# YujiaoShi/HighlyAccurate

Measured on AMD Instinct MI355X. Metric: image-pairs/sec through N-iter LM pose loop, KITTI shapes, higher is better.
Workload: dtype bf16; 1 GPU; BASELINE configs[1]: LM_S2GP.forward(mode='test'), sat 512x512, grd 256x1024, VGG-16 two-branch, level 3, 5 LM iters x 3 levels, 3-DoF, random-init weights; pairs_per_gpu=32, global_batch=32, parallelism=batch-sharded x1, no collective

## Files before the change

### highlyaccurate_amd/csrc/common.h

```cpp
#pragma once
#include <hip/hip_runtime.h>
#include <atomic>
#include <stdarg.h>
#include <stdio.h>
#include "../../include/hla.h"

void hla_set_error(const char* fmt, ...);

enum { K_PACK = 0, K_CONV02, K_CONV_NT2, K_CONV_NT2_POOL, K_CONV_NT1, K_CONV_NT1_POOL, K_CONF, K_L2NORM,
       K_LM256, K_LM128, K_LM64, K_LM16, K_LMSOLVE, K_GRIDSAMPLE, K_LMBWD, K_WGRAD, K_ELEMWISE };
void hla_prof_begin(int id, double flops, double bytes, hipStream_t st);
void hla_prof_begin_dyn(int id, double flops, double bytes, hipStream_t st, const int* dev_live, int denom);
void hla_prof_end(hipStream_t st);
bool hla_prof_on();

#ifndef HLA_CONV_STAMPS
#define HLA_CONV_STAMPS 0
#endif
#if HLA_CONV_STAMPS
constexpr int HLA_STAMP_N = 8;
struct HlaStampCfg { unsigned long long* buf; int want; int counter; unsigned grid_x, grid_y; };
extern HlaStampCfg g_hla_stamp;
#endif

#define HLA_CHECK_HIP(expr)                                                              \
  do {                                                                                   \
    hipError_t _e = (expr);                                                              \
    if (_e != hipSuccess) {                                                              \
      hla_set_error("%s failed: %s (%s:%d)", #expr, hipGetErrorString(_e), __FILE__, __LINE__); \
      return HLA_ERR_HIP;                                                                \
    }                                                                                    \
  } while (0)

static inline bool hla_dtype_ok(int dtype) { return dtype == HLA_F32 || dtype == HLA_BF16 || dtype == HLA_F16 || dtype == HLA_F16X3; }

#define HLA_REQUIRE(cond, ...)      \
  do {                              \
    if (!(cond)) {                  \
      hla_set_error(__VA_ARGS__);   \
      return HLA_ERR_ARG;           \
    }                               \
  } while (0)

struct HlaPerDeviceOnce {
  std::atomic<unsigned long long> mask{0};
  template <typename F> hipError_t run(F&& f) {
    int d = 0;
    (void)hipGetDevice(&d);
    const unsigned long long bit = (d >= 0 && d < 64) ? 1ull << d : 0ull;
    if (mask.load(std::memory_order_acquire) & bit) return hipSuccess;
    const hipError_t e = f();
    if (e == hipSuccess) mask.fetch_or(bit, std::memory_order_release);
    return e;
  }
};

static inline size_t hla_align_up(size_t x, size_t a) { return (x + a - 1) / a * a; }

__device__ __forceinline__ float wave_sum_f32(float v) {
#pragma unroll
  for (int o = 32; o > 0; o >>= 1) v += __shfl_xor(v, o, 64);
  return v;
}
__device__ __forceinline__ double wave_sum_f64(double v) {
#pragma unroll
  for (int o = 32; o > 0; o >>= 1) v += __shfl_xor(v, o, 64);
  return v;
}
```

### highlyaccurate_amd/csrc/lm_solve.hip

```cpp
#include "lm_common.h"
#include <cstring>
#include <mutex>

struct SolveArgs {
  const double* part;
  const double* sat_inv;
  const double* grd_inv;
  int nt, part_ld;
  float* pose;
  float* trace_out;
  int trace_stride;
  const float* rand_uv;
  double* normal_eq;
  double* coef;
  const float* R_FL;
  const float* T_FL;
  int B, reinit;
  int optimizer, t;
  double beta1, beta2;
  double* adam;
  const int* in_view;
  LmSolveCfg cfg;
  LmGeom next;
  unsigned* zero_ticket;
  int zero_steps, zero_pose;
  int* reach_clear;
  const int* gate;
};

template <bool COHERENT>
__device__ __forceinline__ void lm_solve_body(const SolveArgs& a, int b, int lane) {
  float su = a.pose[b * 3 + 0], sv = a.pose[b * 3 + 1], th = a.pose[b * 3 + 2];
  if (!a.part) {
    if (a.reach_clear && lane == 0) a.reach_clear[b] = 0;
    if (a.zero_ticket)
      for (int k = lane; k < a.zero_steps; k += 64) a.zero_ticket[(size_t)k * a.B + b] = 0u;
    if (a.zero_pose) {
      su = sv = th = 0.f;
      if (lane < 3) a.pose[b * 3 + lane] = 0.f;
    }
  }

  if (a.part) {
    double s[14];
#pragma unroll
    for (int k = 0; k < 14; ++k) s[k] = 0.0;
    for (int i = lane; i < a.nt; i += 64) {
      const double* p = a.part + ((size_t)b * a.part_ld + i) * PART_N;
#pragma unroll
      for (int k = 0; k < 14; ++k)
        s[k] += COHERENT ? __hip_atomic_load(p + k, __ATOMIC_RELAXED, __HIP_MEMORY_SCOPE_AGENT) : p[k];
    }
#pragma unroll
    for (int k = 0; k < 14; ++k) s[k] = wave_sum_f64(s[k]);

    if (lane == 0) {
      const double as = a.sat_inv ? a.sat_inv[b] : 1.0, ag = a.grd_inv ? a.grd_inv[b] : 1.0;
      s[0] *= as * as; s[1] *= ag * ag;
      for (int k = 2; k < 11; ++k) s[k] *= as * as;
      for (int k = 11; k < 14; ++k) s[k] *= as * ag;
      if (a.normal_eq) {
        for (int k = 0; k < 14; ++k) a.normal_eq[(size_t)b * 16 + k] = s[k];
        a.normal_eq[(size_t)b * 16 + 14] = a.in_view ? (double)a.in_view[b] : 0.0;
        a.normal_eq[(size_t)b * 16 + 15] = 0.0;
      }
      double H[3][3], g[3], Mi[3][3], d[3], ns, ng;
      if (a.optimizer == 0 || a.optimizer == 3) {
        lm_solve_step(a.cfg, s, H, g, Mi, d, ns, ng);
      } else {
        for (int p = 0; p < 3; ++p) d[p] = 2.0 * (s[8 + p] - s[11 + p]);
        if (a.optimizer == 2) {
          double* mv = a.adam + (size_t)b * 6;
          for (int p = 0; p < 3; ++p) {
            const double m = a.beta1 * mv[p] + (1.0 - a.beta1) * d[p];
            const double v = a.beta2 * mv[3 + p] + (1.0 - a.beta2) * d[p] * d[p];
            mv[p] = m; mv[3 + p] = v;
            d[p] = (m / (1.0 - pow(a.beta1, a.t + 1))) / (sqrt(v / (1.0 - pow(a.beta2, a.t + 1))) + 1e-8);
          }
        }
        for (int p = 0; p < 3; ++p) d[p] *= 0.01;
      }
      su = (float)((double)su - d[0]);
      sv = (float)((double)sv - d[1]);
      th = (float)((double)th - d[2]);
      if (a.reinit) {
        const float ru = a.rand_uv[b], rv = a.rand_uv[a.B + b];
        su = (su > -2.5f && su < 2.5f) ? su : ru;
        sv = (sv > -2.5f && sv < 2.5f) ? sv : rv;
      }
      a.pose[b * 3 + 0] = su; a.pose[b * 3 + 1] = sv; a.pose[b * 3 + 2] = th;
      float* tr = a.trace_out + (size_t)b * a.trace_stride;
      tr[0] = su; tr[1] = sv; tr[2] = th;
    }
  }
  if (a.coef && lane == 0)
    lm_coefficients(a.next, su, sv, th, a.R_FL ? a.R_FL + (size_t)b * 9 : nullptr, a.T_FL ? a.T_FL + (size_t)b * 3 : nullptr,
                    a.coef + (size_t)b * COEF_N);
}

__global__ __launch_bounds__(64) void lm_solve(SolveArgs a) {
  if (a.gate && a.gate[blockIdx.x] == 0) return;
  lm_solve_body<false>(a, blockIdx.x, threadIdx.x);
}

struct AccumArgs {
  const void* sat;
  const void* grd;
  const float* conf;
  LmPoints pts;
  const double* coef;
  double* part;
  int A, h, w, row0, npix, TP, nt, part_ld, xcd_affine;
  int b0, nb;
  int hs, rskip;
  const unsigned char* keep;
  unsigned* ticket;
  int col0;
  int* reach_flag;
  const int* gate;
};

typedef float lm_f2 __attribute__((ext_vector_type(2)));
template <typename F> __device__ __forceinline__ lm_f2 lm_pair(const uint4& v, int ep);
template <> __device__ __forceinline__ lm_f2 lm_pair<float>(const uint4& v, int ep) {
  lm_f2 r;
  r.x = __uint_as_float(ep == 0 ? v.x : v.z);
  r.y = __uint_as_float(ep == 0 ? v.y : v.w);
  return r;
}
template <> __device__ __forceinline__ lm_f2 lm_pair<__bf16>(const uint4& v, int ep) {
  const unsigned w = ep == 0 ? v.x : ep == 1 ? v.y : ep == 2 ? v.z : v.w;
  lm_f2 r;
  r.x = __uint_as_float(w << 16);
  r.y = __uint_as_float(w & 0xffff0000u);
  return r;
}
template <> __device__ __forceinline__ lm_f2 lm_pair<_Float16>(const uint4& v, int ep) {
  typedef _Float16 h2 __attribute__((ext_vector_type(2)));
  const unsigned w = ep == 0 ? v.x : ep == 1 ? v.y : ep == 2 ? v.z : v.w;
  const h2 h = __builtin_bit_cast(h2, w);
  lm_f2 r;
  r.x = (float)h[0];
  r.y = (float)h[1];
  return r;
}

#define LM_OCC 6
#define LM_UNROLL(F) (sizeof(F) == 4 ? 2 : 1)
#define FWD_MAX_TP 512
static inline int lm_pick_tile_fwd(int npix) { return npix >= 16384 ? 512 : (npix >= 4096 ? 256 : 128); }
template <int C, bool USE_W, typename F>
__global__ __launch_bounds__(256, LM_OCC) void lm_accum(AccumArgs a, SolveArgs sa) {
  __shared__ PixParam pp[FWD_MAX_TP];
  __shared__ float red[4][14];
  __shared__ double redd[14];
  int b, tile;
  if (!lm_block_map(a.xcd_affine, a.nt, a.nb, b, tile, a.b0)) return;
  if (a.gate && a.gate[b] == 0) return;
  const int t = threadIdx.x;
  const int p0 = tile * a.TP;
  const int np = min(a.TP, a.npix - p0);
  const double* cf = a.coef + (size_t)b * COEF_N;

  for (int tt = t; tt < np; tt += 256) {
    const int p = p0 + tt;
    const int r = a.row0 + p / a.w, c = p % a.w;
    const float cw = USE_W ? a.conf[((size_t)b * a.hs + (r - a.rskip)) * a.w + c] : 1.f;
    float q[3];
    const bool gm = lm_point(a.pts, b, r, c, a.w, q);
    const bool kept = !a.keep || a.keep[p];
    PixParam P = lm_pixel<C>(cf, q, gm, a.A, cw, a.col0, (a.reach_flag && kept) ? a.reach_flag + b : nullptr);
    if (!kept) {
      P.wx0 = P.wx1 = P.wy0 = P.wy1 = 0.f; P.off = a.col0 * C; P.dxo = P.dyo = 0; P.j2u = P.j2v = 0.f; P.gm = P.wt = P.m = 0.f;
    }
    pp[tt] = P;
  }
  __syncthreads();

  const float j0u = (float)cf[8], j0v = (float)cf[9], j1u = (float)cf[10], j1v = (float)cf[11];
  constexpr int EPL = 16 / (int)sizeof(F);
  constexpr int LPP = C / EPL;
  constexpr int PPW = 64 / LPP;
  const int lane = t & 63, wave = t >> 6;
  const int sub = lane / LPP, cl = (lane % LPP) * EPL;
  const F* satb = (const F*)a.sat + (size_t)b * a.A * a.A * C + cl;
  const F* grdb = (const F*)a.grd + ((size_t)b * a.hs * a.w + (size_t)(a.row0 - a.rskip) * a.w + p0) * C + cl;

  float aS = 0, aG = 0, T1 = 0, T2 = 0, T3 = 0, B1 = 0, B2 = 0, Q = 0, U1 = 0, U2 = 0, U3 = 0, V1 = 0, V2 = 0, V3 = 0;

  constexpr int UNR = LM_UNROLL(F);
#pragma unroll UNR
  for (int i = wave * PPW + sub; i < np; i += 4 * PPW) {
    const PixParam P = pp[i];
    const uint4 t00 = *(const uint4*)(satb + P.off);
    const uint4 t01 = *(const uint4*)(satb + P.off + P.dxo);
    const uint4 t10 = *(const uint4*)(satb + P.off + P.dyo);
    const uint4 t11 = *(const uint4*)(satb + P.off + P.dyo + P.dxo);
    const uint4 gg = *(const uint4*)(grdb + (size_t)i * C);
    lm_f2 xx = {0.f, 0.f}, xy = xx, yy = xx, xs = xx, ys = xx, xg = xx, yg = xx, ss2 = xx, gg2 = xx;
#pragma unroll
    for (int ep = 0; ep < EPL / 2; ++ep) {
      const lm_f2 c00 = lm_pair<F>(t00, ep), c01 = lm_pair<F>(t01, ep), c10 = lm_pair<F>(t10, ep), c11 = lm_pair<F>(t11, ep);
      const lm_f2 top = P.wx0 * c00 + P.wx1 * c01;
      const lm_f2 bot = P.wx0 * c10 + P.wx1 * c11;
      const lm_f2 s = P.wy0 * top + P.wy1 * bot;
      const lm_f2 dsy = bot - top;
      const lm_f2 dsx = P.wy0 * (c01 - c00) + P.wy1 * (c11 - c10);
      const lm_f2 g = lm_pair<F>(gg, ep) * P.gm;
      xx += dsx * dsx; xy += dsx * dsy; yy += dsy * dsy;
      xs += dsx * s; ys += dsy * s; xg += dsx * g; yg += dsy * g;
      ss2 += s * s; gg2 += g * g;
    }
    float Sxx = xx.x + xx.y, Sxy = xy.x + xy.y, Syy = yy.x + yy.y, Sxs = xs.x + xs.y, Sys = ys.x + ys.y;
    float Sxg = xg.x + xg.y, Syg = yg.x + yg.y;
    const float Sss = ss2.x + ss2.y, Sgg = gg2.x + gg2.y;
    aS += Sss; aG += Sgg;
    if (USE_W) { Sxx *= P.wt; Sxy *= P.wt; Syy *= P.wt; Sxs *= P.wt; Sys *= P.wt; Sxg *= P.wt; Syg *= P.wt; }
    T1 += Sxx; T2 += Sxy; T3 += Syy;
    const float b1 = P.j2u * Sxx + P.j2v * Sxy, b2 = P.j2u * Sxy + P.j2v * Syy;
    B1 += b1; B2 += b2;
    Q += P.j2u * b1 + P.j2v * b2;
    U1 += Sxs; U2 += Sys; U3 += P.j2u * Sxs + P.j2v * Sys;
    V1 += Sxg; V2 += Syg; V3 += P.j2u * Sxg + P.j2v * Syg;
  }

  float acc[14] = {aS, aG, T1, T2, T3, B1, B2, Q, U1, U2, U3, V1, V2, V3};
#pragma unroll
  for (int k = 0; k < 14; ++k) acc[k] = wave_sum_f32(acc[k]);
  if (lane == 0) {
#pragma unroll
    for (int k = 0; k < 14; ++k) red[wave][k] = acc[k];
  }
  __syncthreads();
  if (t < 14) redd[t] = ((double)red[0][t] + (double)red[1][t]) + ((double)red[2][t] + (double)red[3][t]);
  __syncthreads();
  if (wave != 0) return;
  if (t < PART_N) {
    const double au = (double)j0u, av = (double)j0v, bu = (double)j1u, bv = (double)j1v;
    const double t1 = redd[2], t2 = redd[3], t3 = redd[4], b1 = redd[5], b2 = redd[6];
    double v = 0.0;
    switch (t) {
      case 0: v = redd[0]; break;
      case 1: v = redd[1]; break;
      case 2: v = au * au * t1 + 2.0 * au * av * t2 + av * av * t3; break;
      case 3: v = au * bu * t1 + (au * bv + av * bu) * t2 + av * bv * t3; break;
      case 4: v = au * b1 + av * b2; break;
      case 5: v = bu * bu * t1 + 2.0 * bu * bv * t2 + bv * bv * t3; break;
      case 6: v = bu * b1 + bv * b2; break;
      case 7: v = redd[7]; break;
      case 8: v = au * redd[8] + av * redd[9]; break;
      case 9: v = bu * redd[8] + bv * redd[9]; break;
      case 10: v = redd[10]; break;
      case 11: v = au * redd[11] + av * redd[12]; break;
      case 12: v = bu * redd[11] + bv * redd[12]; break;
      case 13: v = redd[13]; break;
      default: break;
    }
    __hip_atomic_store(a.part + ((size_t)b * a.part_ld + tile) * PART_N + t, v, __ATOMIC_RELAXED, __HIP_MEMORY_SCOPE_AGENT);
  }
  const unsigned old = lm_draw_ticket(a.ticket + b, lane);
  if (old + 1 != (unsigned)a.nt) return;
  lm_solve_body<true>(sa, b, lane);
}

__global__ __launch_bounds__(256) void lm_inview_kernel(const double* __restrict__ coef, LmPoints pts, int w, int A,
                                                        int npix, int* __restrict__ count, int b0) {
  const int b = b0 + blockIdx.y, p = blockIdx.x * 256 + threadIdx.x;
  const double* cf = coef + (size_t)b * COEF_N;
  int in = 0;
  if (p < npix) {
    float q[3];
    (void)lm_point(pts, b, p / w, p % w, w, q);
    const double X = q[0], Y = q[1], Z = q[2];
    const double u = cf[0] * X + cf[1] * Y + cf[2] * Z + cf[3];
    const double v = cf[4] * X + cf[5] * Y + cf[6] * Z + cf[7];
    const double lim = (double)(A - 1);
    in = ((u >= 0.0) && (u <= lim) && (v >= 0.0) && (v <= lim)) ? 1 : 0;
  }
  const unsigned long long m = __ballot(in);
  if ((threadIdx.x & 63) == 0 && m) atomicAdd(count + b, __popcll(m));
}

static size_t ws_layout(const hla_s2g_config* cfg, const hla_s2g_level* lv, int B, size_t* off_coef, size_t* off_pose,
                        size_t* off_part, int* part_ld) {
  int max_nt = 1;
  for (int l = 0; l < cfg->n_levels; ++l) {
    const int npix = (lv[l].h - lv[l].row0) * lv[l].w;
    const int tp = lm_pick_tile_fwd(npix);
    max_nt = max(max_nt, (npix + tp - 1) / tp);
  }
  *part_ld = max_nt;
  size_t o = 0;
  *off_coef = o; o += hla_align_up((size_t)B * COEF_N * sizeof(double), 256);
  *off_pose = o; o += hla_align_up((size_t)B * 3 * sizeof(float), 256);
  *off_part = o; o += hla_align_up((size_t)B * max_nt * PART_N * sizeof(double), 256);
  o += hla_align_up((size_t)B * cfg->n_levels * cfg->n_iters * sizeof(unsigned), 256);
  o += hla_align_up((size_t)B * cfg->n_levels * cfg->n_iters * sizeof(int), 256);
  o += hla_align_up((size_t)B * 6 * sizeof(double), 256);
  return o;
}

extern "C" size_t hla_s2g_workspace_bytes(const hla_s2g_config* cfg, const hla_s2g_level* levels, int B) {
  size_t a, b, c;
  int ld;
  return ws_layout(cfg, levels, B, &a, &b, &c, &ld);
}

template <bool W, typename F>
static void launch_accum_f(int C, dim3 grid, hipStream_t st, const AccumArgs& a, const SolveArgs& sa) {
  switch (C) {
    case 256: hipLaunchKernelGGL((lm_accum<256, W, F>), grid, dim3(256), 0, st, a, sa); break;
    case 128: hipLaunchKernelGGL((lm_accum<128, W, F>), grid, dim3(256), 0, st, a, sa); break;
    case 64: hipLaunchKernelGGL((lm_accum<64, W, F>), grid, dim3(256), 0, st, a, sa); break;
    case 16: hipLaunchKernelGGL((lm_accum<16, W, F>), grid, dim3(256), 0, st, a, sa); break;
  }
}
template <bool W>
static void launch_accum(int C, int feat_dtype, dim3 grid, hipStream_t st, const AccumArgs& a, const SolveArgs& sa) {
  if (feat_dtype == HLA_BF16) launch_accum_f<W, __bf16>(C, grid, st, a, sa);
  else if (feat_dtype == HLA_F16) launch_accum_f<W, _Float16>(C, grid, st, a, sa);
  else launch_accum_f<W, float>(C, grid, st, a, sa);
}

int hla_s2g_validate(const char* who, const hla_s2g_config* cfg, const hla_s2g_level* lv, const float* R_FL,
                     const float* T_FL, int B) {
  HLA_REQUIRE(cfg && lv, "%s: null argument", who);
  HLA_REQUIRE(B > 0 && cfg->n_levels >= 1 && cfg->n_levels <= 4 && cfg->n_iters >= 1, "%s: bad sizes", who);
  HLA_REQUIRE(cfg->dof >= 1 && cfg->dof <= 3, "%s: dof must be 1..3", who);
  HLA_REQUIRE(cfg->proj == 0, "%s: cfg->proj selects the projection of hla_g2s_* only (must be 0 here)", who);
  HLA_REQUIRE(!cfg->ford || (R_FL && T_FL), "%s: Ford mode needs R_FL and T_FL", who);
  HLA_REQUIRE(cfg->reach_mode == 0 || (!strcmp(who, "hla_s2g_lm_solve") && cfg->reach_mode >= 1 && cfg->reach_mode <= 2 && cfg->reach_flag),
              "%s: cfg->reach_mode is 0, or 1 / 2 with reach_flag in hla_s2g_lm_solve", who);
  for (int l = 0; l < cfg->n_levels; ++l) {
    const int C = lv[l].C;
    HLA_REQUIRE(C == 256 || C == 128 || C == 64 || C == 16, "%s: unsupported channel count %d", who, C);
    HLA_REQUIRE(lv[l].feat_dtype == HLA_F32 || lv[l].feat_dtype == HLA_BF16 || lv[l].feat_dtype == HLA_F16,
                "%s: level %d feat_dtype must be HLA_F32, HLA_BF16 or HLA_F16", who, l);
    HLA_REQUIRE(lv[l].sat_feat && lv[l].grd_feat && lv[l].xyz, "%s: level %d has null maps", who, l);
    HLA_REQUIRE(!cfg->using_weight || lv[l].grd_conf, "%s: using_weight needs grd_conf", who);
    HLA_REQUIRE(lv[l].row0 >= 0 && lv[l].row0 < lv[l].h, "%s: bad row0", who);
    HLA_REQUIRE(lv[l].grd_row_skip >= 0 && lv[l].grd_row_skip <= lv[l].row0, "%s: grd_row_skip must be in [0,row0]", who);
    HLA_REQUIRE((size_t)lv[l].A * lv[l].A * C < (1u << 31), "%s: satellite map too large", who);
    HLA_REQUIRE(cfg->reach_mode != 1 || (cfg->reach_col0[l] >= 0 && cfg->reach_col0[l] < lv[l].A),
                "%s: cfg->reach_col0[%d] must be in [0, A)", who, l);
    if (lv[l].depth) {
// ... 13 lines not shown
constexpr int LM_SPLIT_MIN = 16;
static_assert(LM_GROUPS >= 2 && LM_GROUPS <= 4 && LM_SPLIT_MIN > 8, "a batch of up to 8 samples is one XCD octet and never splits");

struct LmSideStreams {
  std::mutex mu;
  bool ready = false, failed = false;
  hipStream_t side[LM_GROUPS] = {};
  hipEvent_t fork = nullptr, join[LM_GROUPS] = {};
};
static LmSideStreams g_lm_side[64];

static bool lm_side_create(LmSideStreams& S) {
  if (S.ready || S.failed) return S.ready;
  hipError_t r = hipEventCreateWithFlags(&S.fork, hipEventDisableTiming);
  for (int g = 1; g < LM_GROUPS && r == hipSuccess; ++g) {
    r = hipStreamCreateWithFlags(&S.side[g], hipStreamNonBlocking);
    if (r == hipSuccess) r = hipEventCreateWithFlags(&S.join[g], hipEventDisableTiming);
  }
  if (r != hipSuccess) {
    (void)hipGetLastError();
    if (S.fork) (void)hipEventDestroy(S.fork);
    for (int g = 1; g < LM_GROUPS; ++g) {
      if (S.join[g]) (void)hipEventDestroy(S.join[g]);
      if (S.side[g]) (void)hipStreamDestroy(S.side[g]);
    }
    S.failed = true;
    return false;
  }
  S.ready = true;
  return true;
}

extern "C" int hla_s2g_lm_solve(const hla_s2g_config* cfg, const hla_s2g_level* lv, const float* R_FL,
                                const float* T_FL, const float* pose0, const float* rand_uv, float* trace,
                                double* normal_eq, void* workspace, size_t workspace_bytes, int B,
                                hla_stream_t stream) {
  HLA_REQUIRE(trace && workspace, "hla_s2g_lm_solve: null argument");
  const int rc = hla_s2g_validate("hla_s2g_lm_solve", cfg, lv, R_FL, T_FL, B);
  if (rc) return rc;
  HLA_REQUIRE(cfg->optimizer >= 0 && cfg->optimizer <= 3, "hla_s2g_lm_solve: optimizer must be 0 (LM), 1 (SGD), 2 (ADAM) or 3 (GN)");
  HLA_REQUIRE(cfg->optimizer == 0 || !cfg->level_first, "hla_s2g_lm_solve: SGD / ADAM / GN exist for the iteration-first loop only");
  HLA_REQUIRE(cfg->optimizer != 3 || cfg->ford, "hla_s2g_lm_solve: GN_update exists in the Ford model only");
  const bool newton = cfg->optimizer == 0 || cfg->optimizer == 3;
  const bool reinit = (cfg->ford || cfg->dof == 3) && newton;
  HLA_REQUIRE(!reinit || rand_uv, "hla_s2g_lm_solve: rand_uv required");
  size_t oc, op, opart;
  int part_ld;
  const size_t need = ws_layout(cfg, lv, B, &oc, &op, &opart, &part_ld);
  if (workspace_bytes < need) {
    hla_set_error("hla_s2g_lm_solve: workspace %zu < %zu", workspace_bytes, need);
    return HLA_ERR_WORKSPACE;
  }
  hipStream_t st = (hipStream_t)stream;
  char* ws = (char*)workspace;
  double* coef = (double*)(ws + oc);
  float* pose = (float*)(ws + op);
  double* part = (double*)(ws + opart);

  if (pose0) HLA_CHECK_HIP(hipMemcpyAsync(pose, pose0, (size_t)B * 3 * sizeof(float), hipMemcpyDeviceToDevice, st));

  const int L = cfg->n_levels, N = cfg->n_iters, steps = L * N;
  auto step_level = [&](int k) { return cfg->level_first ? k / N : k % L; };
  auto step_iter = [&](int k) { return cfg->level_first ? k % N : k / L; };
  auto geom = [&](int l) {
    LmGeom g{};
    g.ford = cfg->ford; g.lat = cfg->shift_range_lat; g.lon = cfg->shift_range_lon; g.rot = cfg->rotation_range;
    g.mpp = lv[l].meter_per_pixel; g.ctr = lv[l].centre;
    return g;
  };

  double* adam = (double*)(ws + need - hla_align_up((size_t)B * 6 * sizeof(double), 256));
  int* in_view = (int*)((char*)adam - hla_align_up((size_t)B * steps * sizeof(int), 256));
  unsigned* ticket = (unsigned*)((char*)in_view - hla_align_up((size_t)B * steps * sizeof(unsigned), 256));
  const bool count = cfg->count_in_view && normal_eq;
  if (count) HLA_CHECK_HIP(hipMemsetAsync(in_view, 0, (size_t)B * steps * sizeof(int), st));
  if (cfg->optimizer == 2) HLA_CHECK_HIP(hipMemsetAsync(adam, 0, (size_t)B * 6 * sizeof(double), st));
  SolveArgs sa{};
  sa.optimizer = cfg->optimizer; sa.beta1 = cfg->beta1; sa.beta2 = cfg->beta2; sa.adam = adam;
  sa.pose = pose; sa.B = B; sa.part_ld = part_ld; sa.reinit = reinit ? 1 : 0; sa.R_FL = R_FL; sa.T_FL = T_FL;
  sa.cfg.gn = cfg->optimizer == 3 ? 1 : 0;
  sa.cfg.dof = cfg->dof; sa.cfg.use_hessian = sa.cfg.gn ? 0 : cfg->use_hessian;
  for (int i = 0; i < 3; ++i) sa.cfg.lam[i] = sa.cfg.gn ? 0.0 : cfg->damping[i];
  sa.coef = coef;

  sa.part = nullptr; sa.next = geom(step_level(0));
  sa.zero_ticket = ticket; sa.zero_steps = steps; sa.zero_pose = pose0 ? 0 : 1;
  sa.reach_clear = cfg->reach_mode == 1 ? cfg->reach_flag : nullptr;
  sa.gate = cfg->reach_mode == 2 ? cfg->reach_flag : nullptr;
  hipLaunchKernelGGL(lm_solve, dim3(B), dim3(64), 0, st, sa);
  sa.zero_ticket = nullptr; sa.zero_steps = 0; sa.zero_pose = 0; sa.reach_clear = nullptr;

  int ng = 1, gb0[LM_GROUPS + 1] = {0};
  LmSideStreams* side = nullptr;
  std::unique_lock<std::mutex> side_lock;
  if (B >= LM_SPLIT_MIN && !hla_prof_on() && cfg->reach_mode != 2) {
    hipStreamCaptureStatus cap = hipStreamCaptureStatusNone;
    int d = -1;
    if (hipStreamIsCapturing(st, &cap) != hipSuccess || hipGetDevice(&d) != hipSuccess) { (void)hipGetLastError(); d = -1; }
    if (cap == hipStreamCaptureStatusNone && d >= 0 && d < 64) {
      side_lock = std::unique_lock<std::mutex>(g_lm_side[d].mu);
      if (lm_side_create(g_lm_side[d])) side = &g_lm_side[d];
      else side_lock.unlock();
    }
  }
  if (side) {
    const int oct = (B + 7) / 8;
    ng = oct < LM_GROUPS ? oct : LM_GROUPS;
    for (int g = 0; g < ng; ++g) gb0[g + 1] = gb0[g] + 8 * (oct / ng + (g < oct % ng ? 1 : 0));
  }
  gb0[ng] = B;
  hipStream_t gst[LM_GROUPS];
  gst[0] = st;
  int forked = 0;
  hipError_t err = hipSuccess;
  if (ng > 1) {
    err = hipEventRecord(side->fork, st);
    for (int g = 1; g < ng && err == hipSuccess; ++g) {
      gst[g] = side->side[g];
      err = hipStreamWaitEvent(gst[g], side->fork, 0);
      if (err == hipSuccess) forked = g;
    }
  }

  for (int k = 0; k < steps && err == hipSuccess; ++k) {
    const int l = step_level(k), it = step_iter(k);
    const hla_s2g_level& v = lv[l];
    AccumArgs aa{};
    aa.sat = v.sat_feat; aa.grd = v.grd_feat; aa.conf = v.grd_conf; aa.pts = lm_points_of(v); aa.coef = coef; aa.part = part;
    aa.A = v.A; aa.h = v.h; aa.w = v.w; aa.row0 = v.row0; aa.npix = (v.h - v.row0) * v.w;
    aa.hs = v.h - v.grd_row_skip; aa.rskip = v.grd_row_skip;
    aa.keep = cfg->keep ? cfg->keep + (size_t)k * cfg->keep_stride : nullptr;
    aa.TP = lm_pick_tile_fwd(aa.npix); aa.nt = (aa.npix + aa.TP - 1) / aa.TP; aa.part_ld = part_ld;
    aa.xcd_affine = (B >= 8) ? 1 : 0;
    aa.ticket = ticket + (size_t)k * B;
    if (cfg->reach_mode == 1) { aa.col0 = cfg->reach_col0[l]; aa.reach_flag = cfg->reach_flag; }
    aa.gate = sa.gate;
    sa.t = k;
    sa.part = part; sa.nt = aa.nt; sa.sat_inv = v.sat_inv_norm; sa.grd_inv = v.grd_inv_norm;
    sa.trace_out = trace + ((size_t)it * L + l) * 3; sa.trace_stride = N * L * 3;
    sa.rand_uv = reinit ? rand_uv + (size_t)k * 2 * B : nullptr;
    sa.normal_eq = normal_eq ? normal_eq + (size_t)k * B * 16 : nullptr;
    sa.in_view = count ? in_view + (size_t)k * B : nullptr;
    if (k + 1 < steps) { sa.coef = coef; sa.next = geom(step_level(k + 1)); }
    else sa.coef = nullptr;
    const double esz = v.feat_dtype == HLA_F32 ? 4.0 : 2.0;
    for (int g = 0; g < ng; ++g) {
      hipStream_t gs = gst[g];
      aa.b0 = gb0[g]; aa.nb = gb0[g + 1] - gb0[g];
      if (count)
        hipLaunchKernelGGL(lm_inview_kernel, dim3((v.h * v.w + 255) / 256, aa.nb), dim3(256), 0, gs, coef, aa.pts, v.w, v.A, v.h * v.w,
                           in_view + (size_t)k * B, aa.b0);
      const int nblk = aa.xcd_affine ? 8 * ((aa.nb + 7) / 8) * aa.nt : aa.nb * aa.nt;
      hla_prof_begin(v.C == 256 ? K_LM256 : v.C == 128 ? K_LM128 : v.C == 64 ? K_LM64 : K_LM16, 0,
                     (double)aa.nb * ((double)v.A * v.A + (double)aa.npix) * v.C * esz, gs);
      if (cfg->using_weight && newton) launch_accum<true>(v.C, v.feat_dtype, dim3(nblk), gs, aa, sa);
      else launch_accum<false>(v.C, v.feat_dtype, dim3(nblk), gs, aa, sa);
      hla_prof_end(gs);
    }
  }
  for (int g = 1; g <= forked; ++g) {
    hipError_t e = hipEventRecord(side->join[g], gst[g]);
    if (e == hipSuccess) e = hipStreamWaitEvent(st, side->join[g], 0);
    if (err == hipSuccess) err = e;
  }
  HLA_CHECK_HIP(err);
  HLA_CHECK_HIP(hipGetLastError());
// ... 3 lines not shown
```

### highlyaccurate_amd/csrc/prof.hip

```cpp
#include "common.h"
#include <mutex>
#include <vector>

namespace {
struct Rec { int id; double flops, bytes; hipEvent_t a, b; int live_slot, live_denom; };
std::vector<Rec> g_recs;
std::mutex g_mu;
bool g_on = false;
constexpr int kLiveSlots = 4096;
int* g_live = nullptr;
int g_live_used = 0;
const char* kNames[HLA_PROF_NKERNELS] = {
    "pack_weights_kernel", "conv02_kernel", "conv3x3_kernel<MT4,NT2>", "conv3x3_kernel<MT4,NT2,pool>",
    "conv3x3_kernel<MT4,NT1>", "conv3x3_kernel<MT4,NT1,pool>", "conf_kernel", "inv_norm+scale_kernel",
    "lm_accum<256>", "lm_accum<128>", "lm_accum<64>", "lm_accum<16>", "lm_solve", "grid_sample_kernel", "lm_bwd_accum", "wgrad_kernel", "elementwise_bwd"};
}

bool hla_prof_on() { return g_on; }

void hla_prof_begin(int id, double flops, double bytes, hipStream_t st) { hla_prof_begin_dyn(id, flops, bytes, st, nullptr, 0); }

void hla_prof_begin_dyn(int id, double flops, double bytes, hipStream_t st, const int* dev_live, int denom) {
  if (!g_on) return;
  Rec r{id, flops, bytes, nullptr, nullptr, -1, denom};
  std::lock_guard<std::mutex> lk(g_mu);
  if (dev_live && denom > 0) {
    if (!g_live && hipHostMalloc((void**)&g_live, kLiveSlots * sizeof(int), hipHostMallocDefault) != hipSuccess) g_live = nullptr;
    if (g_live && g_live_used < kLiveSlots) {
      r.live_slot = g_live_used++;
      g_live[r.live_slot] = denom;
      (void)hipMemcpyAsync(g_live + r.live_slot, dev_live, sizeof(int), hipMemcpyDeviceToHost, st);
    }
  }
  (void)hipEventCreate(&r.a);
  (void)hipEventCreate(&r.b);
  (void)hipEventRecord(r.a, st);
  g_recs.push_back(r);
}

void hla_prof_end(hipStream_t st) {
  if (!g_on) return;
  std::lock_guard<std::mutex> lk(g_mu);
  if (!g_recs.empty()) (void)hipEventRecord(g_recs.back().b, st);
}

extern "C" int hla_prof_enable(int on) {
  std::lock_guard<std::mutex> lk(g_mu);
  g_on = on != 0;
  return HLA_OK;
}

extern "C" const char* hla_prof_kernel_name(int id) { return (id >= 0 && id < HLA_PROF_NKERNELS) ? kNames[id] : "?"; }

extern "C" int hla_prof_fetch(hla_prof_record* out, int max_records, int* n_out) {
  std::lock_guard<std::mutex> lk(g_mu);
  int n = 0;
  for (auto& r : g_recs) {
    float ms = 0.f;
    if (hipEventSynchronize(r.b) == hipSuccess) (void)hipEventElapsedTime(&ms, r.a, r.b);
    double frac = 1.0;
    if (r.live_slot >= 0 && g_live) {
      const int live = g_live[r.live_slot];
      frac = live < 0 ? 0.0 : (live > r.live_denom ? 1.0 : (double)live / r.live_denom);
    }
    if (out && n < max_records) { out[n].kernel_id = r.id; out[n].flops = r.flops * frac; out[n].bytes = r.bytes * frac; out[n].ms = ms; ++n; }
    (void)hipEventDestroy(r.a);
    (void)hipEventDestroy(r.b);
  }
  g_recs.clear();
  g_live_used = 0;
  if (n_out) *n_out = n;
  return HLA_OK;
}

#if HLA_CONV_STAMPS
HlaStampCfg g_hla_stamp = {nullptr, -1, 0, 0, 0};
extern "C" int hla_debug_conv_stamps(void* buf, int want) { g_hla_stamp.buf = (unsigned long long*)buf; g_hla_stamp.want = want; g_hla_stamp.counter = 0; return 0; }
extern "C" int hla_debug_conv_stamps_grid(unsigned* gx, unsigned* gy) { *gx = g_hla_stamp.grid_x; *gy = g_hla_stamp.grid_y; return 0; }
#endif

typedef __attribute__((ext_vector_type(8))) __bf16 pk_bf16x8;
typedef __attribute__((ext_vector_type(8))) _Float16 pk_f16x8;
typedef __attribute__((ext_vector_type(16))) float pk_f32x16;
template <int F16>
static __global__ __launch_bounds__(256, 2) void mfma_burn_kernel(const uint4* __restrict__ src, float* __restrict__ out, int iters) {
  const int t = threadIdx.x;
  uint4 a[4], b[4];
#pragma unroll
  for (int i = 0; i < 4; ++i) { a[i] = src[(t * 8 + i) & 4095]; b[i] = src[(t * 8 + 4 + i) & 4095]; }
  pk_f32x16 acc[8];
#pragma unroll
  for (int i = 0; i < 8; ++i)
#pragma unroll
    for (int r = 0; r < 16; ++r) acc[i][r] = 0.f;
  for (int it = 0; it < iters; ++it) {
#pragma unroll
    for (int i = 0; i < 8; ++i) {
      if (F16)
// ... 63 lines not shown
```

### include/hla.h

```cpp
#ifndef HLA_H
#define HLA_H

#include <stddef.h>
#include <stdint.h>

#ifdef __cplusplus
extern "C" {
#endif

typedef void* hla_stream_t;

typedef enum hla_status {
  HLA_OK = 0,
  HLA_ERR_ARG = -1,
  HLA_ERR_HIP = -2,
  HLA_ERR_WORKSPACE = -3
} hla_status;

typedef enum hla_dtype {
  HLA_F32 = 0,
  HLA_BF16 = 1,
  HLA_F16 = 2,
  HLA_F16X3 = 3
} hla_dtype;
// ... 131 lines not shown
  int proj;
  int reach_mode;
  int* reach_flag;
  int reach_col0[4];
} hla_s2g_config;

size_t hla_s2g_workspace_bytes(const hla_s2g_config* cfg, const hla_s2g_level* levels, int B);

int hla_s2g_lm_solve(const hla_s2g_config* cfg, const hla_s2g_level* levels, const float* R_FL,
                     const float* T_FL, const float* pose0, const float* rand_uv, float* trace,
                     double* normal_eq, void* workspace, size_t workspace_bytes, int B, hla_stream_t stream);

size_t hla_s2g_pose_score_workspace_bytes(const hla_s2g_config* cfg, const hla_s2g_level* level, int B, int K);
int hla_s2g_pose_score(const hla_s2g_config* cfg, const hla_s2g_level* level, const float* R_FL, const float* T_FL,
                       const float* poses, int K, double* sums, float* cost, void* workspace, size_t workspace_bytes, int B,
                       hla_stream_t stream);

size_t hla_g2s_workspace_bytes(const hla_s2g_config* cfg, const hla_s2g_level* levels, int B);
int hla_g2s_lm_solve(const hla_s2g_config* cfg, const hla_s2g_level* levels, const float* camera_k, int ori_h, int ori_w,
                     const float* pose0, float* trace, double* normal_eq, void* workspace, size_t workspace_bytes,
                     int B, hla_stream_t stream);

size_t hla_g2s_pose_score_workspace_bytes(const hla_s2g_config* cfg, const hla_s2g_level* level, int B, int K);
int hla_g2s_pose_score(const hla_s2g_config* cfg, const hla_s2g_level* level, const float* camera_k, int ori_h, int ori_w,
                       const float* poses, int K, double* sums, float* cost, void* workspace, size_t workspace_bytes, int B,
                       hla_stream_t stream);

typedef struct hla_s2g_level_grad {
  float* d_sat_feat;
  float* d_grd_feat;
  float* d_grd_conf;
} hla_s2g_level_grad;

size_t hla_s2g_bwd_workspace_bytes(const hla_s2g_config* cfg, const hla_s2g_level* levels, int B);

int hla_s2g_lm_solve_bwd(const hla_s2g_config* cfg, const hla_s2g_level* levels, const hla_s2g_level_grad* grads,
                         const float* R_FL, const float* T_FL, const float* pose0, const float* trace,
                         const double* normal_eq, const float* d_trace, double* d_damping, void* workspace,
                         size_t workspace_bytes, int B, hla_stream_t stream);

size_t hla_g2s_bwd_workspace_bytes(const hla_s2g_config* cfg, const hla_s2g_level* levels, int B);
int hla_g2s_lm_solve_bwd(const hla_s2g_config* cfg, const hla_s2g_level* levels, const hla_s2g_level_grad* grads,
                         const float* camera_k, int ori_h, int ori_w, const float* pose0, const float* trace,
                         const double* normal_eq, const float* d_trace, double* d_damping, void* workspace,
                         size_t workspace_bytes, int B, hla_stream_t stream);


typedef struct hla_fill_region {
  void* ptr;
  size_t chunk_bytes, stride_bytes;
  int n_chunks;
} hla_fill_region;
int hla_zero_fill(const hla_fill_region* regions, int n_regions, int max_blocks, hla_stream_t stream);

enum { HLA_POSE_LOSS_F32 = 0, HLA_POSE_LOSS_F64 = 1 };
typedef struct hla_pose_loss_args {
  const float* x[3];
  long long x_stride[3][3];
  const void* gt[3];
  long long gt_stride[3];
  double coe[3];
  int B, N, L;
  int gt_dtype;
} hla_pose_loss_args;
int hla_pose_loss(const hla_pose_loss_args* args, void* out, hla_stream_t stream);
int hla_pose_loss_bwd(const hla_pose_loss_args* args, const void* const g_out[9], float* const dx[3],
                      const long long dx_stride[3][3], hla_stream_t stream);

size_t hla_orien_corr_workspace_bytes(int B, int H, int W, int C, int S);
int hla_orien_corr(const float* P1, const float* grd_feat, const double* p1_inv_norm, const double* grd_inv_norm, double* dot,
                   double* E, double* gnorm, float* corr, void* workspace, size_t workspace_bytes, int B, int H, int W, int C,
                   int S, hla_stream_t stream);
int hla_orien_corr_bwd(const float* P1, const float* grd_feat, const double* p1_inv_norm, const double* grd_inv_norm,
                       const double* dot, const double* E, const double* gnorm, const float* d_corr, float* d_P1,
                       float* d_grd_feat, void* workspace, size_t workspace_bytes, int B, int H, int W, int C, int S,
                       hla_stream_t stream);
int hla_orien_window_bwd(const float* optical, const float* d_out, double* acc, float* d_image, int N, int C, int IH, int IW,
                         int H, int W, hla_stream_t stream);
int hla_orien_triplet_loss(const float* corr, const float* gt_heading, long long gt_stride, double rotation_range,
                           double degree_per_pixel, float* loss, int accumulate, int B, int S, hla_stream_t stream);
int hla_orien_triplet_loss_bwd(const float* corr, const float* gt_heading, long long gt_stride, double rotation_range,
                               double degree_per_pixel, const float* g_loss, float* d_corr, int B, int S, hla_stream_t stream);

#define HLA_PROF_NKERNELS 17
typedef struct hla_prof_record {
  int kernel_id;
  float ms;
  double flops;
  double bytes;
} hla_prof_record;
int hla_prof_enable(int on);
const char* hla_prof_kernel_name(int kernel_id);
int hla_prof_fetch(hla_prof_record* out, int max_records, int* n_out);
int hla_prof_mfma_peak(int dtype, int data, float ms_target, float* tflops_out, hla_stream_t stream);

#ifdef __cplusplus
}
#endif
#endif
```

Before: 6008 pairs/s.

## Fuse LM repair iterations into one persistent per-pair kernel

Adds a persistent kernel, lm_repair_loop, that runs every LM step across all levels inside a single launch with one 1024-thread block per pair. Each block keeps pose and coefficients in shared memory and processes tiles in four groups. It replaces the per-step lm_accum launches and ticket-based solves when reach_mode==2, Newton is used, no weights or counting are active, and features are 16-bit. This removes launch and grid-synchronisation overhead, but only B blocks are active, which risks low GPU occupancy. The tile body is factored into a shared include, and its bilinear interpolation now uses explicit packed FMAs.

```diff
diff --git a/highlyaccurate_amd/csrc/common.h b/highlyaccurate_amd/csrc/common.h
--- a/highlyaccurate_amd/csrc/common.h
+++ b/highlyaccurate_amd/csrc/common.h
@@ -8,7 +8,7 @@
 void hla_set_error(const char* fmt, ...);
 
 enum { K_PACK = 0, K_CONV02, K_CONV_NT2, K_CONV_NT2_POOL, K_CONV_NT1, K_CONV_NT1_POOL, K_CONF, K_L2NORM,
-       K_LM256, K_LM128, K_LM64, K_LM16, K_LMSOLVE, K_GRIDSAMPLE, K_LMBWD, K_WGRAD, K_ELEMWISE };
+       K_LM256, K_LM128, K_LM64, K_LM16, K_LMSOLVE, K_GRIDSAMPLE, K_LMBWD, K_WGRAD, K_ELEMWISE, K_LMREPAIR };
 void hla_prof_begin(int id, double flops, double bytes, hipStream_t st);
 void hla_prof_begin_dyn(int id, double flops, double bytes, hipStream_t st, const int* dev_live, int denom);
 void hla_prof_end(hipStream_t st);
diff --git a/highlyaccurate_amd/csrc/lm_solve.hip b/highlyaccurate_amd/csrc/lm_solve.hip
--- a/highlyaccurate_amd/csrc/lm_solve.hip
+++ b/highlyaccurate_amd/csrc/lm_solve.hip
@@ -28,16 +28,16 @@
   const int* gate;
 };
 
-template <bool COHERENT>
-__device__ __forceinline__ void lm_solve_body(const SolveArgs& a, int b, int lane) {
-  float su = a.pose[b * 3 + 0], sv = a.pose[b * 3 + 1], th = a.pose[b * 3 + 2];
+template <bool COHERENT, bool LOCAL = false>
+__device__ __forceinline__ void lm_solve_body(const SolveArgs& a, int b, int lane, float* lpose = nullptr, double* lcoef = nullptr) {
+  float su = LOCAL ? lpose[0] : a.pose[b * 3 + 0], sv = LOCAL ? lpose[1] : a.pose[b * 3 + 1], th = LOCAL ? lpose[2] : a.pose[b * 3 + 2];
   if (!a.part) {
     if (a.reach_clear && lane == 0) a.reach_clear[b] = 0;
     if (a.zero_ticket)
       for (int k = lane; k < a.zero_steps; k += 64) a.zero_ticket[(size_t)k * a.B + b] = 0u;
     if (a.zero_pose) {
       su = sv = th = 0.f;
-      if (lane < 3) a.pose[b * 3 + lane] = 0.f;
+      if (lane < 3) (LOCAL ? lpose[lane] : a.pose[b * 3 + lane]) = 0.f;
     }
   }
 
@@ -88,14 +88,15 @@
         su = (su > -2.5f && su < 2.5f) ? su : ru;
         sv = (sv > -2.5f && sv < 2.5f) ? sv : rv;
       }
-      a.pose[b * 3 + 0] = su; a.pose[b * 3 + 1] = sv; a.pose[b * 3 + 2] = th;
+      if (LOCAL) { lpose[0] = su; lpose[1] = sv; lpose[2] = th; }
+      else { a.pose[b * 3 + 0] = su; a.pose[b * 3 + 1] = sv; a.pose[b * 3 + 2] = th; }
       float* tr = a.trace_out + (size_t)b * a.trace_stride;
       tr[0] = su; tr[1] = sv; tr[2] = th;
     }
   }
-  if (a.coef && lane == 0)
+  if ((LOCAL ? lcoef : a.coef) && lane == 0)
     lm_coefficients(a.next, su, sv, th, a.R_FL ? a.R_FL + (size_t)b * 9 : nullptr, a.T_FL ? a.T_FL + (size_t)b * 3 : nullptr,
-                    a.coef + (size_t)b * COEF_N);
+                    LOCAL ? lcoef : a.coef + (size_t)b * COEF_N);
 }
 
 __global__ __launch_bounds__(64) void lm_solve(SolveArgs a) {
@@ -121,6 +122,7 @@
 };
 
 typedef float lm_f2 __attribute__((ext_vector_type(2)));
+__device__ __forceinline__ lm_f2 lm_fma2(float w, lm_f2 x, lm_f2 y) { return __builtin_elementwise_fma(lm_f2{w, w}, x, y); }
 template <typename F> __device__ __forceinline__ lm_f2 lm_pair(const uint4& v, int ep);
 template <> __device__ __forceinline__ lm_f2 lm_pair<float>(const uint4& v, int ep) {
   lm_f2 r;
@@ -149,6 +151,7 @@
 #define LM_UNROLL(F) (sizeof(F) == 4 ? 2 : 1)
 #define FWD_MAX_TP 512
 static inline int lm_pick_tile_fwd(int npix) { return npix >= 16384 ? 512 : (npix >= 4096 ? 256 : 128); }
+
 template <int C, bool USE_W, typename F>
 __global__ __launch_bounds__(256, LM_OCC) void lm_accum(AccumArgs a, SolveArgs sa) {
   __shared__ PixParam pp[FWD_MAX_TP];
@@ -158,109 +161,110 @@
   if (!lm_block_map(a.xcd_affine, a.nt, a.nb, b, tile, a.b0)) return;
   if (a.gate && a.gate[b] == 0) return;
   const int t = threadIdx.x;
-  const int p0 = tile * a.TP;
-  const int np = min(a.TP, a.npix - p0);
-  const double* cf = a.coef + (size_t)b * COEF_N;
-
-  for (int tt = t; tt < np; tt += 256) {
-    const int p = p0 + tt;
-    const int r = a.row0 + p / a.w, c = p % a.w;
-    const float cw = USE_W ? a.conf[((size_t)b * a.hs + (r - a.rskip)) * a.w + c] : 1.f;
-    float q[3];
-    const bool gm = lm_point(a.pts, b, r, c, a.w, q);
-    const bool kept = !a.keep || a.keep[p];
-    PixParam P = lm_pixel<C>(cf, q, gm, a.A, cw, a.col0, (a.reach_flag && kept) ? a.reach_flag + b : nullptr);
-    if (!kept) {
-      P.wx0 = P.wx1 = P.wy0 = P.wy1 = 0.f; P.off = a.col0 * C; P.dxo = P.dyo = 0; P.j2u = P.j2v = 0.f; P.gm = P.wt = P.m = 0.f;
-    }
-    pp[tt] = P;
-  }
-  __syncthreads();
-
-  const float j0u = (float)cf[8], j0v = (float)cf[9], j1u = (float)cf[10], j1v = (float)cf[11];
-  constexpr int EPL = 16 / (int)sizeof(F);
-  constexpr int LPP = C / EPL;
-  constexpr int PPW = 64 / LPP;
-  const int lane = t & 63, wave = t >> 6;
-  const int sub = lane / LPP, cl = (lane % LPP) * EPL;
-  const F* satb = (const F*)a.sat + (size_t)b * a.A * a.A * C + cl;
-  const F* grdb = (const F*)a.grd + ((size_t)b * a.hs * a.w + (size_t)(a.row0 - a.rskip) * a.w + p0) * C + cl;
-
-  float aS = 0, aG = 0, T1 = 0, T2 = 0, T3 = 0, B1 = 0, B2 = 0, Q = 0, U1 = 0, U2 = 0, U3 = 0, V1 = 0, V2 = 0, V3 = 0;
-
-  constexpr int UNR = LM_UNROLL(F);
-#pragma unroll UNR
-  for (int i = wave * PPW + sub; i < np; i += 4 * PPW) {
-    const PixParam P = pp[i];
-    const uint4 t00 = *(const uint4*)(satb + P.off);
-    const uint4 t01 = *(const uint4*)(satb + P.off + P.dxo);
-    const uint4 t10 = *(const uint4*)(satb + P.off + P.dyo);
-    const uint4 t11 = *(const uint4*)(satb + P.off + P.dyo + P.dxo);
-    const uint4 gg = *(const uint4*)(grdb + (size_t)i * C);
-    lm_f2 xx = {0.f, 0.f}, xy = xx, yy = xx, xs = xx, ys = xx, xg = xx, yg = xx, ss2 = xx, gg2 = xx;
-#pragma unroll
-    for (int ep = 0; ep < EPL / 2; ++ep) {
-      const lm_f2 c00 = lm_pair<F>(t00, ep), c01 = lm_pair<F>(t01, ep), c10 = lm_pair<F>(t10, ep), c11 = lm_pair<F>(t11, ep);
-      const lm_f2 top = P.wx0 * c00 + P.wx1 * c01;
-      const lm_f2 bot = P.wx0 * c10 + P.wx1 * c11;
-      const lm_f2 s = P.wy0 * top + P.wy1 * bot;
-      const lm_f2 dsy = bot - top;
-      const lm_f2 dsx = P.wy0 * (c01 - c00) + P.wy1 * (c11 - c10);
-      const lm_f2 g = lm_pair<F>(gg, ep) * P.gm;
-      xx += dsx * dsx; xy += dsx * dsy; yy += dsy * dsy;
-      xs += dsx * s; ys += dsy * s; xg += dsx * g; yg += dsy * g;
-      ss2 += s * s; gg2 += g * g;
-    }
-    float Sxx = xx.x + xx.y, Sxy = xy.x + xy.y, Syy = yy.x + yy.y, Sxs = xs.x + xs.y, Sys = ys.x + ys.y;
-    float Sxg = xg.x + xg.y, Syg = yg.x + yg.y;
-    const float Sss = ss2.x + ss2.y, Sgg = gg2.x + gg2.y;
-    aS += Sss; aG += Sgg;
-    if (USE_W) { Sxx *= P.wt; Sxy *= P.wt; Syy *= P.wt; Sxs *= P.wt; Sys *= P.wt; Sxg *= P.wt; Syg *= P.wt; }
-    T1 += Sxx; T2 += Sxy; T3 += Syy;
-    const float b1 = P.j2u * Sxx + P.j2v * Sxy, b2 = P.j2u * Sxy + P.j2v * Syy;
-    B1 += b1; B2 += b2;
-    Q += P.j2u * b1 + P.j2v * b2;
-    U1 += Sxs; U2 += Sys; U3 += P.j2u * Sxs + P.j2v * Sys;
-    V1 += Sxg; V2 += Syg; V3 += P.j2u * Sxg + P.j2v * Syg;
-  }
-
-  float acc[14] = {aS, aG, T1, T2, T3, B1, B2, Q, U1, U2, U3, V1, V2, V3};
-#pragma unroll
-  for (int k = 0; k < 14; ++k) acc[k] = wave_sum_f32(acc[k]);
-  if (lane == 0) {
-#pragma unroll
-    for (int k = 0; k < 14; ++k) red[wave][k] = acc[k];
-  }
-  __syncthreads();
-  if (t < 14) redd[t] = ((double)red[0][t] + (double)red[1][t]) + ((double)red[2][t] + (double)red[3][t]);
-  __syncthreads();
-  if (wave != 0) return;
-  if (t < PART_N) {
-    const double au = (double)j0u, av = (double)j0v, bu = (double)j1u, bv = (double)j1v;
-    const double t1 = redd[2], t2 = redd[3], t3 = redd[4], b1 = redd[5], b2 = redd[6];
-    double v = 0.0;
-    switch (t) {
-      case 0: v = redd[0]; break;
-      case 1: v = redd[1]; break;
-      case 2: v = au * au * t1 + 2.0 * au * av * t2 + av * av * t3; break;
-      case 3: v = au * bu * t1 + (au * bv + av * bu) * t2 + av * bv * t3; break;
-      case 4: v = au * b1 + av * b2; break;
-      case 5: v = bu * bu * t1 + 2.0 * bu * bv * t2 + bv * bv * t3; break;
-      case 6: v = bu * b1 + bv * b2; break;
-      case 7: v = redd[7]; break;
-      case 8: v = au * redd[8] + av * redd[9]; break;
-      case 9: v = bu * redd[8] + bv * redd[9]; break;
-      case 10: v = redd[10]; break;
-      case 11: v = au * redd[11] + av * redd[12]; break;
-      case 12: v = bu * redd[11] + bv * redd[12]; break;
-      case 13: v = redd[13]; break;
-      default: break;
-    }
-    __hip_atomic_store(a.part + ((size_t)b * a.part_ld + tile) * PART_N + t, v, __ATOMIC_RELAXED, __HIP_MEMORY_SCOPE_AGENT);
-  }
+  constexpr bool active = true;
+#define LM_TILE_COEF (a.coef + (size_t)b * COEF_N)
+#define LM_TILE_BEFORE_PUBLISH if (wave != 0) return;
+#include "lm_tile_body.h"
+#undef LM_TILE_COEF
+#undef LM_TILE_BEFORE_PUBLISH
   const unsigned old = lm_draw_ticket(a.ticket + b, lane);
   if (old + 1 != (unsigned)a.nt) return;
   lm_solve_body<true>(sa, b, lane);
+}
+
+struct RepairLevel {
+  const void* sat; const void* grd;
+  LmPoints pts;
+  const double* sat_inv; const double* grd_inv;
+  int A, h, w, row0, npix, TP, nt, hs, rskip, C;
+  double mpp, ctr;
+};
+struct RepairArgs {
+  RepairLevel lv[4];
+  SolveArgs sa;
+  double* part;
+  const unsigned char* keep; size_t keep_stride;
+  float* trace; const float* rand_uv; double* normal_eq;
+  int L, N, level_first;
+};
+#define LM_REPAIR_GROUPS 4
+
+template <typename F>
+__global__ __launch_bounds__(256 * LM_REPAIR_GROUPS) void lm_repair_loop(RepairArgs ra) {
+  __shared__ PixParam s_pp[LM_REPAIR_GROUPS][FWD_MAX_TP];
+  __shared__ float s_red[LM_REPAIR_GROUPS][4][14];
+  __shared__ double s_redd[LM_REPAIR_GROUPS][14];
+  __shared__ double s_cf[COEF_N];
+  __shared__ float s_pose[3];
+  const int b = blockIdx.x;
+  if (ra.sa.gate[b] == 0) return;
+  const int wt = threadIdx.x, vg = wt >> 8, vt = wt & 255;
+  const int L = ra.L, N = ra.N, steps = L * N;
+  auto step_level = [&](int k) { return ra.level_first ? k / N : k % L; };
+
+  if (wt < 3) s_pose[wt] = ra.sa.pose[b * 3 + wt];
+  __syncthreads();
+  if (wt < 64) {
+    SolveArgs sa = ra.sa;
+    const RepairLevel& n = ra.lv[step_level(0)];
+    sa.part = nullptr; sa.next.mpp = n.mpp; sa.next.ctr = n.ctr;
+    lm_solve_body<false, true>(sa, b, wt, s_pose, s_cf);
+  }
+  __syncthreads();
+
+  for (int k = 0; k < steps; ++k) {
+    const int l = step_level(k), it = ra.level_first ? k % N : k / L;
+    const RepairLevel& lv = ra.lv[l];
+    AccumArgs a{};
+    a.sat = lv.sat; a.grd = lv.grd; a.pts = lv.pts; a.part = ra.part;
+    a.A = lv.A; a.h = lv.h; a.w = lv.w; a.row0 = lv.row0; a.npix = lv.npix; a.TP = lv.TP; a.nt = lv.nt; a.part_ld = ra.sa.part_ld;
+    a.hs = lv.hs; a.rskip = lv.rskip;
+    a.keep = ra.keep ? ra.keep + (size_t)k * ra.keep_stride : nullptr;
+    for (int tile0 = 0; tile0 < lv.nt; tile0 += LM_REPAIR_GROUPS) {
+      const int tile = tile0 + vg;
+      const bool active = tile < lv.nt;
+      constexpr bool USE_W = false;
+      const int t = vt;
+      PixParam* const pp = s_pp[vg];
+      float (*const red)[14] = s_red[vg];
+      double* const redd = s_redd[vg];
+#define LM_TILE_COEF s_cf
+#define LM_TILE_BEFORE_PUBLISH
+      switch (lv.C) {
+        case 256: {
+          constexpr int C = 256;
+#include "lm_tile_body.h"
+        } break;
+        case 128: {
+          constexpr int C = 128;
+#include "lm_tile_body.h"
+        } break;
+        default: {
+          constexpr int C = 64;
+#include "lm_tile_body.h"
+        } break;
+      }
+#undef LM_TILE_COEF
+#undef LM_TILE_BEFORE_PUBLISH
+    }
+    asm volatile("s_waitcnt vmcnt(0)" ::: "memory");
+    __syncthreads();
+    if (wt < 64) {
+      SolveArgs sa = ra.sa;
+      sa.t = k;
+      sa.part = ra.part; sa.nt = lv.nt; sa.sat_inv = lv.sat_inv; sa.grd_inv = lv.grd_inv;
+      sa.trace_out = ra.trace + ((size_t)it * L + l) * 3; sa.trace_stride = N * L * 3;
+      sa.rand_uv = ra.sa.reinit ? ra.rand_uv + (size_t)k * 2 * ra.sa.B : nullptr;
+      sa.normal_eq = ra.normal_eq ? ra.normal_eq + (size_t)k * ra.sa.B * 16 : nullptr;
+      if (k + 1 < steps) {
+        const RepairLevel& n = ra.lv[step_level(k + 1)];
+        sa.next.mpp = n.mpp; sa.next.ctr = n.ctr;
+      }
+      lm_solve_body<true, true>(sa, b, wt, s_pose, k + 1 < steps ? s_cf : nullptr);
+    }
+    __syncthreads();
+  }
+  if (wt < 3) ra.sa.pose[b * 3 + wt] = s_pose[wt];
 }
 
 __global__ __launch_bounds__(256) void lm_inview_kernel(const double* __restrict__ coef, LmPoints pts, int w, int A,
@@ -440,6 +444,35 @@
   sa.cfg.dof = cfg->dof; sa.cfg.use_hessian = sa.cfg.gn ? 0 : cfg->use_hessian;
   for (int i = 0; i < 3; ++i) sa.cfg.lam[i] = sa.cfg.gn ? 0.0 : cfg->damping[i];
   sa.coef = coef;
+
+  bool repair = cfg->reach_mode == 2 && newton && !cfg->using_weight && !count && lv[0].feat_dtype != HLA_F32;
+  for (int l = 0; l < L && repair; ++l) repair = lv[l].C != 16 && lv[l].feat_dtype == lv[0].feat_dtype;
+  if (repair) {
+    RepairArgs ra{};
+    for (int l = 0; l < L; ++l) {
+      const hla_s2g_level& v = lv[l];
+      RepairLevel& r = ra.lv[l];
+      r.sat = v.sat_feat; r.grd = v.grd_feat; r.pts = lm_points_of(v); r.sat_inv = v.sat_inv_norm; r.grd_inv = v.grd_inv_norm;
+      r.A = v.A; r.h = v.h; r.w = v.w; r.row0 = v.row0; r.npix = (v.h - v.row0) * v.w;
+      r.TP = lm_pick_tile_fwd(r.npix); r.nt = (r.npix + r.TP - 1) / r.TP;
+      r.hs = v.h - v.grd_row_skip; r.rskip = v.grd_row_skip; r.C = v.C;
+      r.mpp = v.meter_per_pixel; r.ctr = v.centre;
+    }
+    ra.sa = sa;
+    ra.sa.next = geom(0);
+    ra.sa.zero_pose = pose0 ? 0 : 1;
+    ra.sa.gate = cfg->reach_flag;
+    ra.part = part;
+    ra.keep = cfg->keep; ra.keep_stride = (size_t)cfg->keep_stride;
+    ra.trace = trace; ra.rand_uv = rand_uv; ra.normal_eq = normal_eq;
+    ra.L = L; ra.N = N; ra.level_first = cfg->level_first;
+    hla_prof_begin(K_LMREPAIR, 0, 0, st);
+    if (lv[0].feat_dtype == HLA_BF16) hipLaunchKernelGGL(lm_repair_loop<__bf16>, dim3(B), dim3(256 * LM_REPAIR_GROUPS), 0, st, ra);
+    else hipLaunchKernelGGL(lm_repair_loop<_Float16>, dim3(B), dim3(256 * LM_REPAIR_GROUPS), 0, st, ra);
+    hla_prof_end(st);
+    HLA_CHECK_HIP(hipGetLastError());
+    return HLA_OK;
+  }
 
   sa.part = nullptr; sa.next = geom(step_level(0));
   sa.zero_ticket = ticket; sa.zero_steps = steps; sa.zero_pose = pose0 ? 0 : 1;
diff --git a/highlyaccurate_amd/csrc/lm_tile_body.h b/highlyaccurate_amd/csrc/lm_tile_body.h
--- /dev/null
+++ b/highlyaccurate_amd/csrc/lm_tile_body.h
@@ -0,0 +1,103 @@
+#if !defined(LM_TILE_COEF) || !defined(LM_TILE_BEFORE_PUBLISH)
+#error "lm_tile_body.h is a text fragment of lm_accum / lm_repair_loop (csrc/lm_solve.hip): define LM_TILE_COEF and LM_TILE_BEFORE_PUBLISH"
+#endif
+  const int p0 = tile * a.TP;
+  const int np = active ? min(a.TP, a.npix - p0) : 0;
+  const double* cf = LM_TILE_COEF;
+
+  for (int tt = t; tt < np; tt += 256) {
+    const int p = p0 + tt;
+    const int r = a.row0 + p / a.w, c = p % a.w;
+    const float cw = USE_W ? a.conf[((size_t)b * a.hs + (r - a.rskip)) * a.w + c] : 1.f;
+    float q[3];
+    const bool gm = lm_point(a.pts, b, r, c, a.w, q);
+    const bool kept = !a.keep || a.keep[p];
+    PixParam P = lm_pixel<C>(cf, q, gm, a.A, cw, a.col0, (a.reach_flag && kept) ? a.reach_flag + b : nullptr);
+    if (!kept) {
+      P.wx0 = P.wx1 = P.wy0 = P.wy1 = 0.f; P.off = a.col0 * C; P.dxo = P.dyo = 0; P.j2u = P.j2v = 0.f; P.gm = P.wt = P.m = 0.f;
+    }
+    pp[tt] = P;
+  }
+  __syncthreads();
+
+  const float j0u = (float)cf[8], j0v = (float)cf[9], j1u = (float)cf[10], j1v = (float)cf[11];
+  constexpr int EPL = 16 / (int)sizeof(F);
+  constexpr int LPP = C / EPL;
+  constexpr int PPW = 64 / LPP;
+  const int lane = t & 63, wave = t >> 6;
+  const int sub = lane / LPP, cl = (lane % LPP) * EPL;
+  const F* satb = (const F*)a.sat + (size_t)b * a.A * a.A * C + cl;
+  const F* grdb = (const F*)a.grd + ((size_t)b * a.hs * a.w + (size_t)(a.row0 - a.rskip) * a.w + p0) * C + cl;
+
+  float aS = 0, aG = 0, T1 = 0, T2 = 0, T3 = 0, B1 = 0, B2 = 0, Q = 0, U1 = 0, U2 = 0, U3 = 0, V1 = 0, V2 = 0, V3 = 0;
+
+  constexpr int UNR = LM_UNROLL(F);
+#pragma unroll UNR
+  for (int i = wave * PPW + sub; i < np; i += 4 * PPW) {
+    const PixParam P = pp[i];
+    const uint4 t00 = *(const uint4*)(satb + P.off);
+    const uint4 t01 = *(const uint4*)(satb + P.off + P.dxo);
+    const uint4 t10 = *(const uint4*)(satb + P.off + P.dyo);
+    const uint4 t11 = *(const uint4*)(satb + P.off + P.dyo + P.dxo);
+    const uint4 gg = *(const uint4*)(grdb + (size_t)i * C);
+    lm_f2 xx = {0.f, 0.f}, xy = xx, yy = xx, xs = xx, ys = xx, xg = xx, yg = xx, ss2 = xx, gg2 = xx;
+#pragma unroll
+    for (int ep = 0; ep < EPL / 2; ++ep) {
+      const lm_f2 c00 = lm_pair<F>(t00, ep), c01 = lm_pair<F>(t01, ep), c10 = lm_pair<F>(t10, ep), c11 = lm_pair<F>(t11, ep);
+      const lm_f2 top = lm_fma2(P.wx0, c00, P.wx1 * c01);
+      const lm_f2 bot = lm_fma2(P.wx0, c10, P.wx1 * c11);
+      const lm_f2 s = lm_fma2(P.wy0, top, P.wy1 * bot);
+      const lm_f2 dsy = bot - top;
+      const lm_f2 dsx = lm_fma2(P.wy0, c01 - c00, P.wy1 * (c11 - c10));
+      const lm_f2 g = lm_pair<F>(gg, ep) * P.gm;
+      xx += dsx * dsx; xy += dsx * dsy; yy += dsy * dsy;
+      xs += dsx * s; ys += dsy * s; xg += dsx * g; yg += dsy * g;
+      ss2 += s * s; gg2 += g * g;
+    }
+    float Sxx = xx.x + xx.y, Sxy = xy.x + xy.y, Syy = yy.x + yy.y, Sxs = xs.x + xs.y, Sys = ys.x + ys.y;
+    float Sxg = xg.x + xg.y, Syg = yg.x + yg.y;
+    const float Sss = ss2.x + ss2.y, Sgg = gg2.x + gg2.y;
+    aS += Sss; aG += Sgg;
+    if (USE_W) { Sxx *= P.wt; Sxy *= P.wt; Syy *= P.wt; Sxs *= P.wt; Sys *= P.wt; Sxg *= P.wt; Syg *= P.wt; }
+    T1 += Sxx; T2 += Sxy; T3 += Syy;
+    const float b1 = P.j2u * Sxx + P.j2v * Sxy, b2 = P.j2u * Sxy + P.j2v * Syy;
+    B1 += b1; B2 += b2;
+    Q += P.j2u * b1 + P.j2v * b2;
+    U1 += Sxs; U2 += Sys; U3 += P.j2u * Sxs + P.j2v * Sys;
+    V1 += Sxg; V2 += Syg; V3 += P.j2u * Sxg + P.j2v * Syg;
+  }
+
+  float acc[14] = {aS, aG, T1, T2, T3, B1, B2, Q, U1, U2, U3, V1, V2, V3};
+#pragma unroll
+  for (int k = 0; k < 14; ++k) acc[k] = wave_sum_f32(acc[k]);
+  if (lane == 0) {
+#pragma unroll
+    for (int k = 0; k < 14; ++k) red[wave][k] = acc[k];
+  }
+  __syncthreads();
+  if (t < 14) redd[t] = ((double)red[0][t] + (double)red[1][t]) + ((double)red[2][t] + (double)red[3][t]);
+  __syncthreads();
+  LM_TILE_BEFORE_PUBLISH
+  if (active && t < PART_N) {
+    const double au = (double)j0u, av = (double)j0v, bu = (double)j1u, bv = (double)j1v;
+    const double t1 = redd[2], t2 = redd[3], t3 = redd[4], b1 = redd[5], b2 = redd[6];
+    double v = 0.0;
+    switch (t) {
+      case 0: v = redd[0]; break;
+      case 1: v = redd[1]; break;
+      case 2: v = au * au * t1 + 2.0 * au * av * t2 + av * av * t3; break;
+      case 3: v = au * bu * t1 + (au * bv + av * bu) * t2 + av * bv * t3; break;
+      case 4: v = au * b1 + av * b2; break;
+      case 5: v = bu * bu * t1 + 2.0 * bu * bv * t2 + bv * bv * t3; break;
+      case 6: v = bu * b1 + bv * b2; break;
+      case 7: v = redd[7]; break;
+      case 8: v = au * redd[8] + av * redd[9]; break;
+      case 9: v = bu * redd[8] + bv * redd[9]; break;
+      case 10: v = redd[10]; break;
+      case 11: v = au * redd[11] + av * redd[12]; break;
+      case 12: v = bu * redd[11] + bv * redd[12]; break;
+      case 13: v = redd[13]; break;
+      default: break;
+    }
+    __hip_atomic_store(a.part + ((size_t)b * a.part_ld + tile) * PART_N + t, v, __ATOMIC_RELAXED, __HIP_MEMORY_SCOPE_AGENT);
+  }
diff --git a/highlyaccurate_amd/csrc/prof.hip b/highlyaccurate_amd/csrc/prof.hip
--- a/highlyaccurate_amd/csrc/prof.hip
+++ b/highlyaccurate_amd/csrc/prof.hip
@@ -13,7 +13,7 @@
 const char* kNames[HLA_PROF_NKERNELS] = {
     "pack_weights_kernel", "conv02_kernel", "conv3x3_kernel<MT4,NT2>", "conv3x3_kernel<MT4,NT2,pool>",
     "conv3x3_kernel<MT4,NT1>", "conv3x3_kernel<MT4,NT1,pool>", "conf_kernel", "inv_norm+scale_kernel",
-    "lm_accum<256>", "lm_accum<128>", "lm_accum<64>", "lm_accum<16>", "lm_solve", "grid_sample_kernel", "lm_bwd_accum", "wgrad_kernel", "elementwise_bwd"};
+    "lm_accum<256>", "lm_accum<128>", "lm_accum<64>", "lm_accum<16>", "lm_solve", "grid_sample_kernel", "lm_bwd_accum", "wgrad_kernel", "elementwise_bwd", "lm_repair_loop"};
 }
 
 bool hla_prof_on() { return g_on; }
diff --git a/include/hla.h b/include/hla.h
--- a/include/hla.h
+++ b/include/hla.h
@@ -237,7 +237,7 @@
 int hla_orien_triplet_loss_bwd(const float* corr, const float* gt_heading, long long gt_stride, double rotation_range,
                                double degree_per_pixel, const float* g_loss, float* d_corr, int B, int S, hla_stream_t stream);
 
-#define HLA_PROF_NKERNELS 17
+#define HLA_PROF_NKERNELS 18
 typedef struct hla_prof_record {
   int kernel_id;
   float ms;
```

New measurement: 6092 pairs/s (median of 6 runs). +1.4%, better.
